# wg-perception/tod

Measured on AMD Instinct MI355X. Metric: frames/sec @ 640x480, 1M-descriptor DB; achieved HBM GB/s on BF-matcher, higher is better.
Workload: dtype fp4 (+-1) x fp4 -> f32 on the matrix cores (exact integers), f32 in the verifier

## Files before the change

tod_amd/csrc/verify.hip:

```cpp
#include <algorithm>
#include <chrono>
#include <atomic>
#include <climits>
#include <cmath>
#include <cstdio>
#include <cstdlib>
#include <cstring>
#include <limits>
#include <map>
#include <memory>
#include <mutex>
#include <thread>
#include <vector>

#include "ctx.h"
#include "depth_rescale.h"
#include "verify_kernels.h"
#include "verify_draw_bits.h"

using namespace tod;

namespace {

#include "verify_launch.h"
#include "verify_prep.h"
#include "verify_draw.h"
#include "verify_clique.h"
#include "verify_eval.h"
#include "verify_growth.h"
#include "verify_sprint.h"


struct VerifyWs {
  DevBuf train, query, qidx, kpxy, phys, samp, bits, sampdeg, nvalid, table, iter_samples, counts, gate_m,
      small, deferred, stacks, kp_bits, clique_adj, adjc_scratch, c_kept, c_offs, c_qpt, c_obj, c_hist, c_goff,
      sprint_status, sprint_stack, c_src, c_cnt;
  HostBuf m_small, m_hist, m_pos, m_counts, m_kp, m_nvalid;
  HostBuf m_sprint, m_sprint_out, m_sprint_kp;
  HostBuf h_small;
};

struct StreamCache;
struct VerifyPool : TodWs {
  static constexpr int kSlot = kWsVerify;
  std::vector<VerifyWs*> slots; std::vector<StreamCache*> streams;
  std::vector<hipEvent_t> side_ev;
  static constexpr size_t kMaxLanes = 17;
  HostBuf args_stage[kMaxLanes]; DevBuf args_dev[kMaxLanes];
  DevBuf kceil; bool kceil_ready = false;
  ~VerifyPool() override;
};
struct SideStreams {
  struct PerDevice {
    std::vector<hipStream_t> st;
    std::atomic<bool> taken[16];
    uint32_t partition = 0;
    PerDevice() { for (auto& t : taken) t.store(false); }
  };
  std::mutex mu;
  std::map<int, PerDevice> by_device;
  hipError_t get(int device, uint32_t n, std::vector<hipStream_t>& out, PerDevice** pd) {
    std::lock_guard<std::mutex> g(mu);
    PerDevice& d = by_device[device];
    const uint32_t part = tod_cu_partition();
    if (d.partition != part) {
      bool in_use = false;
      for (size_t i = 0; i < d.st.size(); ++i) in_use = in_use || d.taken[i].load();
      if (!in_use) {
        for (hipStream_t s0 : d.st) { (void)hipStreamSynchronize(s0); (void)hipStreamDestroy(s0); }
        d.st.clear();
        d.partition = part;
      }
    }
    while (d.st.size() < n) {
      hipStream_t s2;
      const hipError_t e = tod_stream_create(&s2, device, TODHIP_STREAM_LATENCY);
      if (e != hipSuccess) return e;
      d.st.push_back(s2);
    }
    out.assign(d.st.begin(), d.st.begin() + n);
    *pd = &d;
    return hipSuccess;
  }
};
SideStreams g_side_streams;
std::atomic<int> g_batches_in_air{0};

constexpr uint32_t kEvalLdsSmall = 48u * 1024u;
constexpr uint32_t kEvalLdsBig = 160u * 1024u - 512u;
constexpr uint32_t kStackCap = 128u * 1024u;
constexpr uint32_t kMaxEvalWaves = 4096u;

VerifyWs* ws_of(todhip_ctx* ctx, size_t slot = 0) {
  VerifyPool* p = tod_ws<VerifyPool>(ctx);
  while (p->slots.size() <= slot) p->slots.push_back(new VerifyWs());
  return p->slots[slot];
}

struct StreamCache {
  static constexpr uint64_t kSnap = 4096;
  todhip_rng init, gen;
  std::vector<uint32_t> vals;
  std::vector<todhip_rng> snaps;
  explicit StreamCache(const todhip_rng& r) : init(r), gen(r) {}
  bool same_start(const todhip_rng& r) const {
    return r.f == init.f && r.b == init.b && std::memcmp(r.s, init.s, sizeof(init.s)) == 0;
  }
  void extend_to(uint64_t n) {
    while (vals.size() < n) {
      if (vals.size() % kSnap == 0) snaps.push_back(gen);
      vals.push_back(rng_next(gen));
    }
  }
  DevBuf dev;
  uint64_t dev_valid = 0;
  hipError_t ensure_device(uint64_t n, hipStream_t st) {
    extend_to(n);
    if (n <= dev_valid) return hipSuccess;
    const uint64_t want = std::max<uint64_t>(n, 2 * dev_valid);
    extend_to(want);
    if (dev.cap < want * sizeof(uint32_t)) {
      hipError_t e = hipDeviceSynchronize();
      if (e != hipSuccess) return e;
      e = dev.reserve((size_t)want * 2 * sizeof(uint32_t));
      if (e != hipSuccess) return e;
      dev_valid = 0;
    }
    hipError_t e = hipMemcpyAsync(dev.as<uint32_t>() + dev_valid, vals.data() + dev_valid, (size_t)(want - dev_valid) * sizeof(uint32_t),
                                  hipMemcpyHostToDevice, st);
    if (e == hipSuccess) e = hipStreamSynchronize(st);
    if (e == hipSuccess) dev_valid = want;
    return e;
  }
  todhip_rng state_at(uint64_t pos) {
    extend_to(pos + 1);
    todhip_rng g = snaps[pos / kSnap];
    for (uint64_t i = (pos / kSnap) * kSnap; i < pos; ++i) (void)rng_next(g);
    return g;
  }
};

inline double ransac_k(double w) {
  double p_no_outliers = 1.0 - std::pow(w, 3.0);
  p_no_outliers = std::max(std::numeric_limits<double>::epsilon(), p_no_outliers);
  p_no_outliers = std::min(1.0 - std::numeric_limits<double>::epsilon(), p_no_outliers);
  return std::log(1.0 - 0.99) / std::log(p_no_outliers);
}

template <class Launch>
void pick_eval(bool wide, bool deferred, Launch launch) {
  auto extent = [deferred](const EvalArgs& a) { return dim3(deferred ? a.n_deferred : a.it_end - a.it_begin); };
  if (wide) launch(eval_kernel<true, SlotsPtr<EvalArgs>>, eval_kernel<true>, extent);
  else launch(eval_kernel<false, SlotsPtr<EvalArgs>>, eval_kernel<false>, extent);
}

int set_big_lds_once(todhip_ctx* ctx) {
  static std::atomic<bool> done{false};
  if (!done.load(std::memory_order_acquire)) {
    const void* const big[] = {reinterpret_cast<const void*>(eval_kernel<false>), reinterpret_cast<const void*>(eval_kernel<true>),
                               reinterpret_cast<const void*>(eval_kernel<false, SlotsPtr<EvalArgs>>),
                               reinterpret_cast<const void*>(eval_kernel<true, SlotsPtr<EvalArgs>>),
                               reinterpret_cast<const void*>(clique_test_kernel<false>), reinterpret_cast<const void*>(clique_test_kernel<true>),
                               reinterpret_cast<const void*>(chain_kernel)};
    for (const void* f : big) TOD_HIP(hipFuncSetAttribute(f, hipFuncAttributeMaxDynamicSharedMemorySize, (int)kEvalLdsBig));
    TOD_HIP(hipFuncSetAttribute(reinterpret_cast<const void*>(sprint_kernel), hipFuncAttributeMaxDynamicSharedMemorySize,
                                (int)kSprintLds));
    done.store(true, std::memory_order_release);
  }
  return TODHIP_OK;
}

EvalArgs eval_args(const ObjJob& job, VerifyWs* ws, int32_t* counts, uint32_t it_lo, uint32_t it_hi, uint32_t lds_bytes) {
// ... 309 lines not shown
```

tod_amd/csrc/verify_clique.h:

```cpp

struct GateLds {
  u64* adjc;
  u64* mask;
  uint16_t *flist, *cur, *nxt, *tmp;
  uint32_t *C, *deg, *keys;
  uint32_t *S, *SOld, *lbase, *lsize, *lcap;
  uint32_t* trash;
  uint16_t* lstack;
  uint32_t lstack_cap;
};
__host__ __device__ inline uint32_t gate_lds_bytes(uint32_t m) {
  const uint32_t MW = (m + 63u) / 64u, ma = (m + 7u) & ~3u;
  return 8u * m * MW + 8u * MW + 8u * 4u * ma + 4u * 2u * ma + 256u + 64u;
}
__host__ __device__ inline uint32_t gate_small_bytes(uint32_t m) {
  const uint32_t MW = (m + 63u) / 64u, ma = (m + 7u) & ~3u;
  return 8u * MW + 8u * 4u * ma + 4u * 2u * ma + 256u + 64u;
}
template <bool kExt>
__device__ __forceinline__ GateLds gate_carve(unsigned char* base, uint32_t m, uint32_t lds_bytes, u64* ext_adjc = nullptr, uint32_t rows = 0) {
  const uint32_t MW = (m + 63u) / 64u, ma = (m + 7u) & ~3u;
  if (rows == 0u) rows = m;
  unsigned char* const base0 = base;
  GateLds L;
  if constexpr (kExt) { L.adjc = ext_adjc; } else { L.adjc = reinterpret_cast<u64*>(base); base += 8u * rows * MW; }
  L.mask = reinterpret_cast<u64*>(base); base += 8u * MW;
  L.C = reinterpret_cast<uint32_t*>(base); base += 4u * ma;
  L.deg = reinterpret_cast<uint32_t*>(base); base += 4u * ma;
  L.keys = reinterpret_cast<uint32_t*>(base); base += 4u * ma;
  L.S = reinterpret_cast<uint32_t*>(base); base += 4u * ma;
  L.SOld = reinterpret_cast<uint32_t*>(base); base += 4u * ma;
  L.lbase = reinterpret_cast<uint32_t*>(base); base += 4u * ma;
  L.lsize = reinterpret_cast<uint32_t*>(base); base += 4u * ma;
  L.lcap = reinterpret_cast<uint32_t*>(base); base += 4u * ma;
  L.trash = reinterpret_cast<uint32_t*>(base); base += 256u;
  L.flist = reinterpret_cast<uint16_t*>(base); base += 2u * ma;
  L.cur = reinterpret_cast<uint16_t*>(base); base += 2u * ma;
  L.nxt = reinterpret_cast<uint16_t*>(base); base += 2u * ma;
  L.tmp = reinterpret_cast<uint16_t*>(base); base += 2u * ma;
  uint32_t used = ((uint32_t)(base - base0) + 15u) & ~15u;
  L.lstack = reinterpret_cast<uint16_t*>(base0 + used);
  L.lstack_cap = lds_bytes > used ? (lds_bytes - used) / 2u : 0u;
  return L;
}

struct LevelStack { uint16_t* lds; uint32_t lds_cap; uint16_t* glob; };
__device__ __forceinline__ uint16_t stk_get(const LevelStack& s, uint32_t i) {
  return i < s.lds_cap ? s.lds[i] : s.glob[i - s.lds_cap];
}
__device__ __forceinline__ void stk_put(const LevelStack& s, uint32_t i, uint16_t v) {
  if (i < s.lds_cap) s.lds[i] = v; else s.glob[i - s.lds_cap] = v;
}

__device__ __forceinline__ bool row_test(u64 roww, uint32_t h) {
  const u64 wv = shfl64(roww, h >> 6);
  return (wv >> (h & 63u)) & 1ull;
}

constexpr uint32_t kRegChunks = 8;
constexpr uint32_t kSortChunks = 16;

template <uint32_t NCH>
__device__ __forceinline__ void rank_sort_regs(uint16_t* list, const uint32_t* deg, uint32_t r) {
  const uint32_t l = lane_id();
  uint32_t kreg[NCH], rank[NCH];
#pragma unroll
  for (uint32_t c = 0; c < NCH; ++c) {
    const uint32_t i = c * 64u + l;
    kreg[c] = i < r ? ((deg[i] << 16) | list[i]) : 0u;
    rank[c] = 0u;
  }
#pragma unroll
  for (uint32_t cj = 0; cj < NCH; ++cj) {
    const uint32_t cnt = cj * 64u < r ? min(64u, r - cj * 64u) : 0u;
    for (uint32_t lj = 0; lj < cnt; ++lj) {
      const uint32_t kj = rdlane(kreg[cj], lj);
#pragma unroll
      for (uint32_t c = 0; c < NCH; ++c) rank[c] += (kj > kreg[c]) ? 1u : 0u;
    }
  }
  __syncthreads();
#pragma unroll
  for (uint32_t c = 0; c < NCH; ++c)
    if (c * 64u + l < r) list[rank[c]] = (uint16_t)(kreg[c] & 0xFFFFu);
  __syncthreads();
}

template <bool kWide>
__device__ __forceinline__ void rank_sort_desc(uint16_t* list, uint16_t* tmp, const uint32_t* deg, uint32_t r, uint32_t* keys) {
  const uint32_t l = lane_id();
  if (r <= kRegChunks * 64u) {
    switch ((r + 63u) / 64u) {
      case 0: case 1: rank_sort_regs<1>(list, deg, r); break;
      case 2: rank_sort_regs<2>(list, deg, r); break;
      case 3: rank_sort_regs<3>(list, deg, r); break;
      case 4: rank_sort_regs<4>(list, deg, r); break;
      case 5: rank_sort_regs<5>(list, deg, r); break;
      case 6: rank_sort_regs<6>(list, deg, r); break;
      case 7: rank_sort_regs<7>(list, deg, r); break;
      default: rank_sort_regs<8>(list, deg, r); break;
    }
    return;
  }
  if constexpr (kWide) {
    if (r <= kSortChunks * 64u) {
      switch ((r + 63u) / 64u) {
        case 9: rank_sort_regs<9>(list, deg, r); break;
        case 10: rank_sort_regs<10>(list, deg, r); break;
        case 11: rank_sort_regs<11>(list, deg, r); break;
        case 12: rank_sort_regs<12>(list, deg, r); break;
        case 13: case 14: rank_sort_regs<14>(list, deg, r); break;
        default: rank_sort_regs<16>(list, deg, r); break;
      }
      return;
    }
  }
  for (uint32_t i = l; i < r; i += 64u) keys[i] = (deg[i] << 16) | list[i];
  __syncthreads();
  for (uint32_t i0 = 0; i0 < r; i0 += 64u) {
    const uint32_t i = i0 + l;
    const uint32_t mine = i < r ? keys[i] : 0u;
    uint32_t rank = 0;
    for (uint32_t j = 0; j < r; ++j) rank += keys[j] > mine;
    if (i < r) tmp[rank] = (uint16_t)(mine & 0xFFFFu);
  }
  __syncthreads();
  for (uint32_t i = l; i < r; i += 64u) list[i] = tmp[i];
  __syncthreads();
}

__device__ __forceinline__ void degrees_in_list(const GateLds& L, const uint16_t* list, uint32_t r, uint32_t MW) {
  const uint32_t l = lane_id();
  if (l < MW) L.mask[l] = 0ull;
  __syncthreads();
  for (uint32_t i = l; i < r; i += 64u) atomicOr(&L.mask[list[i] >> 6], 1ull << (list[i] & 63u));
  __syncthreads();
  for (uint32_t i = l; i < r; i += 64u) {
    const u64* row = L.adjc + (size_t)list[i] * MW;
    uint32_t d = 0;
    for (uint32_t w = 0; w < MW; ++w) d += (uint32_t)__popcll(row[w] & L.mask[w]);
    L.deg[i] = d;
  }
  __syncthreads();
}

template <uint32_t MWT>
__device__ __forceinline__ bool colour_first_fit64(const GateLds& L, uint16_t* list, uint32_t r) {
  typedef uint32_t u32x16 __attribute__((ext_vector_type(MWT <= 8u ? 16 : 32)));
  const uint32_t l = lane_id();
  u32x16 cls = {};
  uint32_t rec = l << 16;
  uint32_t* const my_trash = L.trash + l;
  for (uint32_t c0 = 0; c0 < r; c0 += 64u) {
    const uint32_t cnt = min(64u, r - c0);
    const uint32_t vmine = (uint32_t)list[min(c0 + l, r - 1u)];
    const uint32_t voff = vmine * (MWT * 8u);
    auto place = [&](const u64 (&row)[MWT], u64 (&next)[MWT], uint32_t li) {
      const uint32_t v = rdlane(vmine, li);
      {
        const u64* g = reinterpret_cast<const u64*>(reinterpret_cast<const unsigned char*>(L.adjc) + rdlane(voff, (li + 1u) & 63u));
#pragma unroll
        for (uint32_t w = 0; w < MWT; ++w) next[w] = g[w];
      }
      uint32_t hit32 = (uint32_t)row[0] & cls[0];
      {
        const uint32_t rh = (uint32_t)(row[0] >> 32), ch = cls[1];
        asm("v_and_or_b32 %0, %1, %2, %0" : "+v"(hit32) : "v"(rh), "v"(ch));
      }
#pragma unroll
      for (uint32_t w = 1; w < MWT; ++w) {
        const uint32_t rl = (uint32_t)row[w], rh = (uint32_t)(row[w] >> 32), cl = cls[2u * w], ch = cls[2u * w + 1u];
        asm("v_and_or_b32 %0, %1, %2, %0" : "+v"(hit32) : "v"(rl), "v"(cl));
        asm("v_and_or_b32 %0, %1, %2, %0" : "+v"(hit32) : "v"(rh), "v"(ch));
      }
      const u64 fm = __ballot(hit32 == 0u);
      const uint32_t below = __builtin_amdgcn_mbcnt_hi((uint32_t)(fm >> 32), __builtin_amdgcn_mbcnt_lo((uint32_t)fm, 0u));
      const uint32_t lw = hit32 == 0u ? below : 1u;
      const bool join = lw == 0u;
      uint32_t* const dst = join ? (L.keys + (c0 + li)) : my_trash;
      *dst = rec;
      rec += join ? 1u : 0u;
      cls[v >> 5] |= join ? (1u << (v & 31u)) : 0u;
    };
    u64 rowA[MWT], rowB[MWT];
    {
      const u64* g = L.adjc + (size_t)rdlane(vmine, 0u) * MWT;
#pragma unroll
      for (uint32_t w = 0; w < MWT; ++w) rowA[w] = g[w];
    }
    uint32_t li = 0;
    for (; li + 2u <= cnt; li += 2u) {
      place(rowA, rowB, li);
      place(rowB, rowA, li + 1u);
    }
    if (li < cnt) place(rowA, rowB, li);
  }
  const uint32_t cnt0 = rec & 0xFFFFu;
  const uint32_t incl0 = wave_incl_scan(cnt0), total0 = uni(__shfl(incl0, 63));
  if (total0 != r) return false;
  const uint32_t base0 = incl0 - cnt0;
  __syncthreads();
  for (uint32_t i = l; i < r + 63u - ((r + 63u) & 63u); i += 64u) {
    const uint32_t rec = i < r ? L.keys[i] : 0u;
    const uint32_t k = rec >> 16;
    const uint32_t b = __shfl(base0, k & 63u);
    if (i < r) {
      const uint32_t pos = b + (rec & 0xFFFFu);
      L.tmp[pos] = list[i];
      L.C[pos] = k + 1u;
    }
  }
  __syncthreads();
  for (uint32_t i = l; i < r; i += 64u) list[i] = L.tmp[i];
  __syncthreads();
  return true;
}

template <uint32_t MWT, bool WIDE>
__device__ __forceinline__ bool colour_first_fit(const GateLds& L, uint16_t* list, uint32_t r) {
  const uint32_t l = lane_id();
  u64 cls0[MWT], cls1[WIDE ? MWT : 1];
#pragma unroll
  for (uint32_t w = 0; w < MWT; ++w) cls0[w] = 0ull;
#pragma unroll
  for (uint32_t w = 0; w < (WIDE ? MWT : 1); ++w) cls1[w] = 0ull;
  uint32_t cnt0 = 0u, cnt1 = 0u;
  bool wide = false, overflow = false;
  for (uint32_t c0 = 0; c0 < r; c0 += 64u) {
    const uint32_t cnt = min(64u, r - c0);
    const uint32_t vmine = (c0 + l) < r ? (uint32_t)list[c0 + l] : 0u;
    uint32_t rec = 0u;
    auto place = [&](const u64 (&row)[MWT], u64 (&next)[MWT], uint32_t li) {
      const uint32_t v = rdlane(vmine, li);
      {
        const u64* g = L.adjc + (size_t)rdlane(vmine, min(li + 1u, cnt - 1u)) * MWT;
#pragma unroll
        for (uint32_t w = 0; w < MWT; ++w) next[w] = g[w];
      }
      u64 hit = 0ull;
#pragma unroll
      for (uint32_t w = 0; w < MWT; ++w) hit |= row[w] & cls0[w];
      const u64 free0 = __ballot(hit == 0ull);
      uint32_t k = 0u;
      bool second = false;
      if (free0 != 0ull) {
        k = (uint32_t)__ffsll((long long)free0) - 1u;
      } else if (WIDE) {
        wide = true; second = true;
        u64 hit1 = 0ull;
#pragma unroll
        for (uint32_t w = 0; w < (WIDE ? MWT : 1); ++w) hit1 |= row[w] & cls1[w];
        const u64 free1 = __ballot(hit1 == 0ull);
        if (free1 == 0ull) overflow = true; else k = (uint32_t)__ffsll((long long)free1) - 1u;
      } else {
        overflow = true;
      }
      const uint32_t vw = v >> 6;
      const u64 bit = 1ull << (v & 63u);
      const uint32_t idx = second ? rdlane(cnt1, k) : rdlane(cnt0, k);
      if (l == k) {
        if (!second) {
          cnt0 += 1u;
#pragma unroll
          for (uint32_t w = 0; w < MWT; ++w)
            if (vw == w) { cls0[w] |= bit; asm volatile("" ::: "memory"); }
        } else if (WIDE) {
          cnt1 += 1u;
#pragma unroll
          for (uint32_t w = 0; w < (WIDE ? MWT : 1); ++w)
            if (vw == w) { cls1[w] |= bit; asm volatile("" ::: "memory"); }
        }
      }
      if (l == li) rec = ((second ? k + 64u : k) << 16) | idx;
    };
    u64 rowA[MWT], rowB[MWT];
    {
      const u64* g = L.adjc + (size_t)rdlane(vmine, 0u) * MWT;
#pragma unroll
      for (uint32_t w = 0; w < MWT; ++w) rowA[w] = g[w];
    }
    uint32_t li = 0;
    for (; li + 2u <= cnt && !overflow; li += 2u) {
      place(rowA, rowB, li);
      place(rowB, rowA, li + 1u);
    }
    if (li < cnt && !overflow) place(rowA, rowB, li);
    if (overflow) return false;
    if (c0 + l < r) L.keys[c0 + l] = rec;
  }
  const uint32_t incl0 = wave_incl_scan(cnt0), total0 = uni(__shfl(incl0, 63));
  const uint32_t base0 = incl0 - cnt0;
  uint32_t base1 = 0u;
  if (wide) { const uint32_t incl1 = wave_incl_scan(cnt1); base1 = total0 + incl1 - cnt1; }
  __syncthreads();
  for (uint32_t i = l; i < r + 63u - ((r + 63u) & 63u); i += 64u) {
    const uint32_t rec = i < r ? L.keys[i] : 0u;
    const uint32_t k = rec >> 16;
    uint32_t b = __shfl(base0, k & 63u);
    if (wide) { const uint32_t b1 = __shfl(base1, k & 63u); b = k >= 64u ? b1 : b; }
    if (i < r) {
      const uint32_t pos = b + (rec & 0xFFFFu);
      L.tmp[pos] = list[i];
      L.C[pos] = k + 1u;
    }
  }
  __syncthreads();
  for (uint32_t i = l; i < r; i += 64u) list[i] = L.tmp[i];
  __syncthreads();
  return true;
}

template <bool kWide>
__device__ __forceinline__ void colour_sort(const GateLds& L, uint16_t* list, uint32_t r, uint32_t MW, uint32_t qmax, uint32_t qsz) {
  const uint32_t l = lane_id();
  const int min_k = max(1, (int)qmax - (int)qsz + 1);
  if (min_k >= 2) {
    if (l == 0) L.C[r - 1] = 0u;
    __syncthreads();
    return;
  }
  if (r <= 2u) {
    if (l == 0) {
      L.C[0] = 1u;
      if (r == 2u) {
        const uint32_t a = list[0], b = list[1];
        L.C[1] = ((L.adjc[(size_t)a * MW + (b >> 6)] >> (b & 63u)) & 1ull) ? 2u : 1u;
      }
    }
    __syncthreads();
    return;
  }
  if (MW <= 8u) {
    bool done = false;
    switch (MW) {
      case 1: done = colour_first_fit64<1>(L, list, r) || colour_first_fit<1, true>(L, list, r); break;
      case 2: done = colour_first_fit64<2>(L, list, r) || colour_first_fit<2, true>(L, list, r); break;
      case 3: done = colour_first_fit64<3>(L, list, r) || colour_first_fit<3, true>(L, list, r); break;
      case 4: done = colour_first_fit64<4>(L, list, r) || colour_first_fit<4, true>(L, list, r); break;
      case 5: done = colour_first_fit64<5>(L, list, r) || colour_first_fit<5, true>(L, list, r); break;
      case 6: done = colour_first_fit64<6>(L, list, r) || colour_first_fit<6, true>(L, list, r); break;
      case 7: done = colour_first_fit64<7>(L, list, r) || colour_first_fit<7, true>(L, list, r); break;
      default: done = colour_first_fit64<8>(L, list, r) || colour_first_fit<8, true>(L, list, r); break;
    }
    if (done) return;
  }
  if constexpr (kWide) {
    if (MW > 8u && MW <= 16u) {
      bool done = false;
      switch (MW) {
        case 9: done = colour_first_fit64<9>(L, list, r) || colour_first_fit<9, true>(L, list, r); break;
        case 10: done = colour_first_fit64<10>(L, list, r) || colour_first_fit<10, true>(L, list, r); break;
        case 11: done = colour_first_fit64<11>(L, list, r) || colour_first_fit<11, true>(L, list, r); break;
        case 12: done = colour_first_fit64<12>(L, list, r) || colour_first_fit<12, true>(L, list, r); break;
        case 13: done = colour_first_fit64<13>(L, list, r) || colour_first_fit<13, true>(L, list, r); break;
        case 14: done = colour_first_fit64<14>(L, list, r) || colour_first_fit<14, true>(L, list, r); break;
        case 15: done = colour_first_fit64<15>(L, list, r) || colour_first_fit<15, true>(L, list, r); break;
        default: done = colour_first_fit64<16>(L, list, r) || colour_first_fit<16, true>(L, list, r); break;
      }
      if (done) return;
    }
  }
  const uint32_t nchunks = (r + 63u) / 64u;
  u64 uncol = 0ull;
  if (l < nchunks) uncol = (l * 64u + 64u <= r) ? ~0ull : ((1ull << (r - l * 64u)) - 1ull);
  uint32_t k = 1, outpos = 0;
  while (__ballot(uncol != 0ull) != 0ull) {
    u64 Q = uncol;
    while (true) {
      const u64 balQ = __ballot(Q != 0ull);
      if (balQ == 0ull) break;
      const uint32_t ll = (uint32_t)__ffsll((long long)balQ) - 1u;
      const u64 wq = shfl64(Q, ll);
      const uint32_t bit = uni((uint32_t)__ffsll((long long)wq) - 1u);
      const uint32_t g = uni(list[ll * 64u + bit]);
      if (l == 0) { L.tmp[outpos] = (uint16_t)g; L.C[outpos] = k; }
      ++outpos;
      if (l == ll) { uncol &= ~(1ull << bit); Q &= ~(1ull << bit); }
      const u64* grow = L.adjc + (size_t)g * MW;
      for (uint32_t c = 0; c < nchunks; ++c) {
        if (!((balQ >> c) & 1ull)) continue;
        const uint32_t pos = c * 64u + l;
        bool adj = false;
        if (pos < r) { const uint32_t h = list[pos]; adj = (grow[h >> 6] >> (h & 63u)) & 1ull; }
        const u64 bal = __ballot(adj);
        if (l == c) Q &= ~bal;
      }
    }
    ++k;
  }
  __syncthreads();
  for (uint32_t i = l; i < r; i += 64u) list[i] = L.tmp[i];
  __syncthreads();
}

template <bool kWide, bool kGate>
__device__ __forceinline__ uint32_t clique_search(GateLds L, uint32_t m, uint32_t minimal_size, uint16_t* gstack, uint32_t stack_cap,
                                  int* err, uint32_t* steps_out, uint32_t* prof = nullptr, const uint16_t* vertices = nullptr) {
  const uint32_t l = lane_id();
  const LevelStack stack = {L.lstack, L.lstack_cap, gstack};
  stack_cap += L.lstack_cap;
  const uint32_t MW = (m + 63u) / 64u;
  uint32_t dmax = 0;
  for (uint32_t i = l; i < m; i += 64u) { L.cur[i] = vertices ? vertices[i] : (uint16_t)i; dmax = max(dmax, L.deg[i]); }
#pragma unroll
  for (int o = 32; o > 0; o >>= 1) dmax = max(dmax, (uint32_t)__shfl_xor((int)dmax, o));
  const uint32_t max_degree = uni(dmax);
  __syncthreads();
  rank_sort_desc<kWide>(L.cur, L.tmp, L.deg, m, L.keys);
  __syncthreads();
  for (uint32_t i = l; i < m; i += 64u) L.C[i] = i < max_degree ? i + 1u : max_degree + 1u;
  for (uint32_t i = l; i < m + 2u; i += 64u) { L.S[i] = 0u; L.SOld[i] = 0u; }
  for (uint32_t i = l; i < m; i += 64u) stk_put(stack, i, L.cur[i]);
  if (l == 0) { L.lbase[1] = 0u; L.lsize[1] = m; L.lcap[1] = m; }
  __syncthreads();

  uint32_t level = 1, qsz = 0, qmax = 0, top = m;
  int all_steps = 1;
  uint32_t pf_isect = 0, pf_sort = 0, pf_col = 0, pf_vfull = 0, pf_big = 0, pf_vbig = 0;
  auto in_lds = [&](uint32_t b, uint32_t n) { return b + n <= stack.lds_cap; };
  uint16_t* cur = in_lds(0u, m) ? stack.lds : L.cur;
  const uint32_t ma = (m + 7u) & ~3u;
  auto frame_word = [&](uint32_t lvl) -> uint32_t { return l < 5u ? (L.S + (size_t)l * ma)[lvl] : 0u; };
  uint32_t sz = m, S_cur = 0u, base_cur = 0u, cap_cur = m;
  while (true) {
    bool ret = false;
    if (sz == 0u) {
      ret = true;
    } else {
      const uint32_t pv = cur[sz - 1u];
      const uint32_t cv = top > 0u ? L.C[top - 1u] : 0u;
      const uint32_t p = uni(pv), c = uni(cv);
      if (qsz + c > qmax) {
        ++qsz;
        const u64* prow = L.adjc + (size_t)p * MW;
        const long long pt0 = prof ? clock64() : 0;
        const uint32_t nb = base_cur + cap_cur;
        const bool in_place = in_lds(nb, sz);
        uint16_t* const nxt = in_place ? stack.lds + nb : (cur == L.cur ? L.nxt : L.cur);
        uint32_t rp = 0;
        for (uint32_t i0 = 0; i0 < sz; i0 += 64u) {
          const uint32_t i = i0 + l;
          uint32_t h = 0;
          bool adj = false;
          if (i < sz) { h = cur[i]; adj = (prow[h >> 6] >> (h & 63u)) & 1ull; }
          const u64 bal = __ballot(adj);
          if (adj) nxt[rp + (uint32_t)__popcll(bal & ((1ull << l) - 1ull))] = (uint16_t)h;
          rp += (uint32_t)__popcll(bal);
        }
        rp = uni(rp);
        __syncthreads();
        const long long pt1 = prof ? clock64() : 0;
        pf_isect += (uint32_t)(pt1 - pt0);
        if constexpr (kGate) {
          if (rp > 0u && qmax < minimal_size && qsz >= minimal_size && (uint32_t)all_steps + rp + 1u <= (uint32_t)kStepCap) { qmax = qsz + 1u; break; }
        }
        if (rp > 0u) {
          if ((uint64_t)S_cur * 40ull < (uint64_t)all_steps) {
            degrees_in_list(L, nxt, rp, MW);
            rank_sort_desc<kWide>(nxt, L.tmp, L.deg, rp, L.keys);
          }
          const long long pt2 = prof ? clock64() : 0;
          pf_sort += (uint32_t)(pt2 - pt1);
          colour_sort<kWide>(L, nxt, rp, MW, qmax, qsz);
          if (prof) {
            const uint32_t dt = (uint32_t)(clock64() - pt2);
            pf_col += dt;
            if ((int)qmax - (int)qsz + 1 < 2) { pf_vfull += rp; if (rp > 64u) { pf_big += dt; pf_vbig += rp; } }
          }
          S_cur += 1u;
          ++all_steps;
          if (all_steps > kStepCap) {
            ret = true;
          } else {
            if (nb + rp > stack_cap) { *err = 1; break; }
            if (!in_place)
              for (uint32_t i = l; i < rp; i += 64u) stk_put(stack, nb + i, nxt[i]);
            const uint32_t child = frame_word(level + 1u);
            if (l == 0) { L.S[level] = S_cur; L.lsize[level] = sz; L.lbase[level] = base_cur; L.lcap[level] = cap_cur; }
            const uint32_t s_child = rdlane(child, 0u), sold_child = rdlane(child, 1u);
            ++level;
            cur = nxt;
            if (qmax >= minimal_size) {
              if (l == 0) L.S[level] = s_child;
              S_cur = s_child; sz = rp; base_cur = nb; cap_cur = rp;
              ret = true;
            } else {
              if (l == 0) L.SOld[level] = S_cur;
              S_cur = s_child + S_cur - sold_child;
              sz = rp; base_cur = nb; cap_cur = rp;
              __syncthreads();
              continue;
            }
          }
        } else {
          if (qsz > qmax) {
            qmax = qsz;
            if (qmax >= minimal_size) {
              if constexpr (kGate) break;
              ret = true;
            }
          }
          if (!ret) --qsz;
        }
      } else {
        ret = true;
      }
      if (!ret) {
        --sz;
        if (top > 0u) --top;
        continue;
      }
    }
    if (level == 1u) break;
    if (l == 0) L.S[level] = S_cur;
    --level;
    --qsz;
    if (top > 0u) --top;
    __syncthreads();
    const uint32_t fw = frame_word(level);
    S_cur = rdlane(fw, 0u); base_cur = rdlane(fw, 2u); sz = rdlane(fw, 3u) - 1u; cap_cur = rdlane(fw, 4u);
    if (in_lds(base_cur, cap_cur)) {
      cur = stack.lds + base_cur;
    } else {
      cur = L.cur;
      for (uint32_t i = l; i < sz; i += 64u) cur[i] = stk_get(stack, base_cur + i);
    }
    __syncthreads();
  }
  if (steps_out) *steps_out = (uint32_t)all_steps;
  if (prof && l == 0) { prof[0] = pf_isect; prof[1] = pf_sort; prof[2] = pf_col; prof[3] = pf_big; prof[4] = pf_vbig; prof[5] = pf_vfull; }
  return qmax;
}

template <bool kGate>
__global__ __launch_bounds__(128) void clique_test_kernel(const u64* adj, uint32_t m, uint32_t minimal_size,
                                                         uint16_t* stack, uint32_t stack_cap, uint32_t lds_bytes,
                                                         uint32_t* out) {
  extern __shared__ __align__(16) unsigned char lds_raw[];
  const uint32_t l = lane_id();
  GateLds L = gate_carve<false>(lds_raw, m, lds_bytes);
  const uint32_t MW = (m + 63u) / 64u;
  for (uint32_t i = l; i < m * MW; i += 64u) L.adjc[i] = adj[i];
  __syncthreads();
  for (uint32_t g = l; g < m; g += 64u) {
    uint32_t d = 0;
    for (uint32_t w = 0; w < MW; ++w) d += (uint32_t)__popcll(L.adjc[(size_t)g * MW + w]);
    L.deg[g] = d;
  }
  __syncthreads();
  int err = 0;
  uint32_t steps = 0;
  const uint32_t q = clique_search<true, kGate>(L, m, minimal_size, stack, stack_cap, &err, &steps);
  if (l == 0) { out[0] = q; out[1] = (uint32_t)err; out[2] = steps; }
}
```

tod_amd/csrc/verify_eval.h:

```cpp

constexpr uint32_t kAdjcScratchWords = 256u * 1024u;

struct EvalArgs {
  ObjJob job;
  const uint32_t* iter_samples;
  uint32_t it_begin, it_end;
  int32_t* counts;
  uint32_t* gate_m;
  uint32_t* work;
  EvalStatus* status;
  uint32_t* deferred;
  uint16_t* stacks;
  uint32_t stack_cap;
  uint32_t lds_bytes;
  uint32_t from_deferred;
  uint32_t n_deferred;
  u64* adjc_scratch;
  uint32_t* dbg;
  uint32_t dbg_stride;
  uint32_t stop_level;
  const uint32_t* n_items_dev;
};

template <bool kExt, bool kWide, int kSlices>
// ... 90 lines not shown
          L.deg[grow] = d;
        }
      }
    } else if (W <= 64u) {
      constexpr uint32_t kRows = 8;
      for (uint32_t g0 = 0; g0 < m; g0 += kRows) {
        u64 rw[kRows];
#pragma unroll
        for (uint32_t j = 0; j < kRows; ++j) {
          const uint32_t g = g0 + j;
          rw[j] = (g < m && l < W) ? job.samp[(size_t)uni(L.flist[g < m ? g : 0u]) * W + l] : 0ull;
        }
#pragma unroll
        for (uint32_t j = 0; j < kRows; ++j) {
          const uint32_t g = g0 + j;
          if (g < m) {
            uint32_t d = 0;
            for (uint32_t c = 0; c < MW; ++c) {
              const uint32_t pos = c * 64u + l;
              const uint32_t h = pos < m ? L.flist[pos] : 0u;
              const bool adj = row_test(rw[j], h) && pos < m;
              const u64 bal = __ballot(adj);
              if (l == 0) L.adjc[(size_t)g * MW + c] = bal;
              d += (uint32_t)__popcll(bal);
            }
            if (l == 0) L.deg[g] = d;
          }
        }
      }
    } else {
      for (uint32_t g = 0; g < m; ++g) {
        const u64* row = job.samp + (size_t)uni(L.flist[g]) * W;
        uint32_t d = 0;
        for (uint32_t c = 0; c < MW; ++c) {
          const uint32_t pos = c * 64u + l;
          bool adj = false;
          if (pos < m) { const uint32_t h = L.flist[pos]; adj = (row[h >> 6] >> (h & 63u)) & 1ull; }
          const u64 bal = __ballot(adj);
          if (l == 0) L.adjc[(size_t)g * MW + c] = bal;
          d += (uint32_t)__popcll(bal);
        }
        if (l == 0) L.deg[g] = d;
      }
    }
  }
  __syncthreads();
  const long long t_adjc = A.dbg ? clock64() : 0;
  if (A.dbg) {
    uint32_t* d = A.dbg + (size_t)it * A.dbg_stride;
    if (l == 0) { d[0] = cnt; d[1] = m; }
    for (uint32_t g = l; g < m && 2u + 2u * g + 1u < A.dbg_stride; g += 64u) { d[2 + 2 * g] = L.flist[g]; d[3 + 2 * g] = L.deg[g]; }
  }
  bool any = false;
  for (uint32_t g = l; g < m; g += 64u) any = any || L.deg[g] > kGateMinimal;
  if (bad_index) {
    result = INT_MIN;
  } else if (A.stop_level != 0u) {
    result = -(int32_t)m;
  } else if (__ballot(any) == 0ull) {
    result = 0;
  } else {
    int err = 0;
    uint32_t steps = 0;
    uint32_t* prof = (A.dbg && A.dbg_stride >= 16u) ? A.dbg + (size_t)it * A.dbg_stride + (A.dbg_stride - 12u) : nullptr;
    const uint32_t q = clique_search<kWide, true>(L, m, kGateMinimal, stack, A.stack_cap, &err, &steps, prof, ident ? L.flist : nullptr);
    if (A.dbg && l == 0 && A.dbg_stride >= 8u) {
      uint32_t* d = A.dbg + (size_t)it * A.dbg_stride + (A.dbg_stride - 6u);
      d[0] = (uint32_t)(t_flist - t_start); d[1] = (uint32_t)(t_adjc - t_flist);
      d[2] = (uint32_t)(clock64() - t_adjc); d[3] = steps; d[4] = q;
    }
    if (err) {
      if (l == 0) atomicExch(&A.status->error, 1u);
      result = INT_MIN;
    } else if (q <= kGateMinimal) {
      result = 0;
    }
    if (l == 0) atomicAdd(&A.status->gate_calls, 1u);
  }
  __syncthreads();
  return result;
}

template <bool kWide, class H = Slots<EvalArgs>>
__global__ __launch_bounds__(128) void eval_kernel(H SL) {
  TOD_LATENCY_PRIO();
  const EvalArgs& A = SL.a[blockIdx.y];
  extern __shared__ __align__(16) unsigned char lds_raw[];
  const uint32_t l = lane_id();
  const ObjJob& job = A.job;
  const uint32_t W = job.W;
  uint16_t* stack = A.stacks + (size_t)blockIdx.x * A.stack_cap;
  uint32_t n_items = A.from_deferred ? A.n_deferred : (A.it_end - A.it_begin);
  if (A.n_items_dev) n_items = min(n_items, uni(*A.n_items_dev));
  {
    const uint32_t item = blockIdx.x;
    if (item >= n_items) return;
    const uint32_t it = uni(A.from_deferred ? A.deferred[item] : (A.it_begin + item));
    const uint32_t s0 = uni(A.iter_samples[3 * it]), s1 = uni(A.iter_samples[3 * it + 1]),
                   s2 = uni(A.iter_samples[3 * it + 2]);
    if (s0 >= job.n || s1 >= job.n || s2 >= job.n) {
      if (l == 0) { atomicExch(&A.status->error, 3u); A.counts[it] = INT_MIN; }
      return;
    }
    typedef WaveBitsT<kWide ? kWPL : 1> Bits;
    Bits P;
    wb_load(P, job.phys + (size_t)s0 * W, W);
    wb_and(P, job.phys + (size_t)s1 * W, W);
    wb_and(P, job.phys + (size_t)s2 * W, W);
    wb_and(P, job.valid, W);
    wb_and(P, job.finite, W);
    const uint32_t cnt = wb_count(P) + 3u;
    int32_t result = (int32_t)cnt;
    uint32_t m_diag = 0;
    if (cnt > kGateMinimal && A.stop_level != 2u) {
      Bits F = P;
      wb_set(F, s0); wb_set(F, s1); wb_set(F, s2);
      wb_and(F, job.deg7, W);
      const uint32_t m = wb_count(F);
      m_diag = m;
      if (m <= kGateMinimal) {
        result = 0;
      } else if (gate_lds_bytes(m) > A.lds_bytes &&
                 !(A.from_deferred && A.adjc_scratch && gate_small_bytes(m) <= A.lds_bytes &&
                   m * ((m + 63u) / 64u) <= kAdjcScratchWords)) {
        if (A.from_deferred) {
          if (l == 0) atomicExch(&A.status->error, 2u);
          result = INT_MIN;
        } else {
          if (l == 0) A.deferred[atomicAdd(&A.status->n_deferred, 1u)] = it;
          result = INT_MIN + 1;
        }
      } else {
        result = gate_lds_bytes(m) > A.lds_bytes ? gate_eval<true, kWide>(A, F, m, it, cnt, lds_raw, stack)
                                                 : gate_eval<false, kWide>(A, F, m, it, cnt, lds_raw, stack);
      }
    }
    if (l == 0) {
      if (result != INT_MIN + 1) A.counts[it] = result;
      if (A.gate_m) A.gate_m[it] = m_diag;
    }
  }
}
```

tod_amd/csrc/verify_kernels.h:

```cpp
#pragma once

#include <hip/hip_runtime.h>

#include <cstddef>
#include <cstdint>

namespace tod {

typedef unsigned long long u64;

constexpr int kMaxWords = 512;
constexpr int kWPL = 8;
constexpr uint32_t kMaxSampleChecks = 1000;
constexpr uint32_t kGateMinimal = 7;
constexpr int kStepCap = 100000;

struct ObjJob {
  uint32_t n, W;
  const float* train;
  const float* query;
  const uint32_t* qidx;
  const float* kpxy;
  u64* phys;
  u64* samp;
  u64* finite;
  u64* valid;
  u64* deg7;
  uint32_t* sampdeg;
};

struct DrawEntry { uint32_t status, consumed, s0, s1, s2, pad; };
enum { DRAW_FAIL = 0, DRAW_OK = 1, DRAW_OVERFLOW = 2 };

struct ChainOut {
  uint32_t n_done;
  uint32_t pos_end;
  uint32_t attempts;
  uint32_t flag;
};

struct EvalStatus {
  uint32_t error;
  uint32_t gate_calls;
  uint32_t n_deferred;
  uint32_t pad_;
  uint32_t detail_g, detail_value, detail_m, detail_it;
};

struct GrowthOut {
  float R[9], T[3];
  uint32_t n_match_inliers;
  uint32_t n_kp_inliers;
  uint32_t passes;
  uint32_t n_model_inliers;
};

struct ClusterCtl {
  uint32_t error, pad1_[3];
  uint32_t n_kept, pad5_[3];
};

template <class Tail>
struct SlotWords {
  uint32_t pad0_;
  ChainOut chain;
  uint32_t prep[3];
  uint32_t eval_work;
  uint32_t pad9_[3];
  EvalStatus eval;
  uint32_t pad20_[12];
  GrowthOut growth;
  uint32_t pad48_[12];
  Tail tail;
};
struct SlotCtlTail { uint32_t pad60_[4]; };
struct SlotMailTail { ClusterCtl cluster; uint32_t pad68_[60]; };
typedef SlotWords<SlotCtlTail> SlotCtl;
typedef SlotWords<SlotMailTail> SlotMail;
constexpr uint32_t kMailSmallWords = 128u;

#define TOD_WORD_AT(T, member, word) static_assert(offsetof(T, member) == (word) * 4u, #T "::" #member " moved")
TOD_WORD_AT(EvalStatus, error, 0); TOD_WORD_AT(EvalStatus, gate_calls, 1); TOD_WORD_AT(EvalStatus, n_deferred, 2);
TOD_WORD_AT(EvalStatus, detail_g, 4); TOD_WORD_AT(EvalStatus, detail_value, 5); TOD_WORD_AT(EvalStatus, detail_m, 6);
TOD_WORD_AT(EvalStatus, detail_it, 7);
TOD_WORD_AT(ClusterCtl, error, 0); TOD_WORD_AT(ClusterCtl, n_kept, 4);
TOD_WORD_AT(SlotCtl, chain, 1); TOD_WORD_AT(SlotCtl, prep, 5); TOD_WORD_AT(SlotCtl, eval_work, 8); TOD_WORD_AT(SlotCtl, eval, 12);
TOD_WORD_AT(SlotCtl, growth, 32); TOD_WORD_AT(SlotCtl, tail, 60);
TOD_WORD_AT(SlotMail, chain, 1); TOD_WORD_AT(SlotMail, prep, 5); TOD_WORD_AT(SlotMail, eval_work, 8); TOD_WORD_AT(SlotMail, eval, 12);
TOD_WORD_AT(SlotMail, growth, 32); TOD_WORD_AT(SlotMail, tail.cluster.error, 60); TOD_WORD_AT(SlotMail, tail.cluster.n_kept, 64);
static_assert(sizeof(EvalStatus) == 8 * 4 && sizeof(ChainOut) == 4 * 4 && sizeof(GrowthOut) == 16 * 4 && sizeof(ClusterCtl) == 8 * 4, "mailbox layout");
static_assert(sizeof(SlotCtl) == 64 * 4 && sizeof(SlotMail) == kMailSmallWords * 4, "mailbox layout");

#undef TOD_WORD_AT

__device__ __forceinline__ uint32_t lane_id() { return threadIdx.x & 63u; }

__device__ __forceinline__ uint32_t uni(uint32_t v) { return (uint32_t)__builtin_amdgcn_readfirstlane((int)v); }

__device__ __forceinline__ uint32_t rdlane(uint32_t v, uint32_t lane) {
  return (uint32_t)__builtin_amdgcn_readlane((int)v, (int)lane);
}
__device__ __forceinline__ u64 rdlane64(u64 v, uint32_t lane) {
  return ((u64)rdlane((uint32_t)(v >> 32), lane) << 32) | rdlane((uint32_t)v, lane);
}

__device__ __forceinline__ uint32_t wave_sum(uint32_t v) {
#pragma unroll
  for (int off = 32; off > 0; off >>= 1) v += __shfl_xor(v, off);
  return uni(v);
}
__device__ __forceinline__ uint32_t wave_incl_scan(uint32_t v) {
  const uint32_t l = lane_id();
#pragma unroll
  for (int d = 1; d < 64; d <<= 1) {
    uint32_t t = __shfl_up(v, d);
    if (l >= (uint32_t)d) v += t;
  }
  return v;
}
__device__ __forceinline__ u64 shfl64(u64 v, uint32_t src) {
  uint32_t lo = __shfl((uint32_t)v, src), hi = __shfl((uint32_t)(v >> 32), src);
  return ((u64)hi << 32) | lo;
}
__device__ __forceinline__ uint32_t nth_set_bit(u64 w, uint32_t n) {
  for (uint32_t i = 0; i < n; ++i) w &= w - 1;
  return (uint32_t)__ffsll((long long)w) - 1u;
}

template <int kSlices = kWPL>
struct WaveBitsT {
  u64 w[kSlices];
};
typedef WaveBitsT<> WaveBits;
template <int kSlices>
__device__ __forceinline__ void wb_load(WaveBitsT<kSlices>& b, const u64* p, uint32_t W) {
  const uint32_t l = lane_id();
#pragma unroll
  for (int j = 0; j < kSlices; ++j) b.w[j] = (j * 64u + l) < W ? p[j * 64u + l] : 0ull;
}
template <int kSlices>
__device__ __forceinline__ void wb_and(WaveBitsT<kSlices>& b, const u64* p, uint32_t W) {
  const uint32_t l = lane_id();
#pragma unroll
  for (int j = 0; j < kSlices; ++j) b.w[j] &= (j * 64u + l) < W ? p[j * 64u + l] : 0ull;
}
template <int kSlices>
__device__ __forceinline__ uint32_t wb_count(const WaveBitsT<kSlices>& b) {
  uint32_t c = 0;
#pragma unroll
  for (int j = 0; j < kSlices; ++j) c += (uint32_t)__popcll(b.w[j]);
  return wave_sum(c);
}
template <int kSlices>
__device__ __forceinline__ void wb_clear(WaveBitsT<kSlices>& b, uint32_t v) {
  const uint32_t word = v >> 6, l = lane_id();
#pragma unroll
  for (int j = 0; j < kSlices; ++j)
    if (word == j * 64u + l) b.w[j] &= ~(1ull << (v & 63u));
}
template <int kSlices>
__device__ __forceinline__ void wb_set(WaveBitsT<kSlices>& b, uint32_t v) {
  const uint32_t word = v >> 6, l = lane_id();
#pragma unroll
  for (int j = 0; j < kSlices; ++j)
    if (word == j * 64u + l) b.w[j] |= (1ull << (v & 63u));
}
template <int kSlices>
__device__ __forceinline__ uint32_t wb_select(const WaveBitsT<kSlices>& b, uint32_t idx) {
  idx = uni(idx);
  uint32_t result = 0xFFFFFFFFu;
#pragma unroll
  for (int j = 0; j < kSlices; ++j) {
    const uint32_t c = (uint32_t)__popcll(b.w[j]);
    const uint32_t incl = wave_incl_scan(c);
    const uint32_t total = uni(__shfl(incl, 63));
    if (result == 0xFFFFFFFFu) {
      if (idx < total) {
        const bool mine = (incl - c) <= idx && idx < incl;
        const u64 bal = __ballot(mine);
        const uint32_t owner = (uint32_t)__ffsll((long long)bal) - 1u;
        const uint32_t bit = mine ? nth_set_bit(b.w[j], idx - (incl - c)) : 0u;
        result = (j * 64u + owner) * 64u + uni(__shfl(bit, owner));
      } else {
        idx -= total;
      }
    }
  }
  return result;
}

__device__ __forceinline__ float dist_sq3(const float* a, const float* b) {
  float t0 = a[0] - b[0], t1 = a[1] - b[1], t2 = a[2] - b[2];
  return t0 * t0 + t1 * t1 + t2 * t2;
}
__device__ __forceinline__ double norm3d(float x, float y, float z) {
  return sqrt((double)x * (double)x + (double)y * (double)y + (double)z * (double)z);
}

}
// ... 1 lines not shown
```

tod_amd/csrc/verify_launch.h:

```cpp

constexpr uint32_t kMaxSlots = 16;
constexpr uint32_t kManySlots = 36;
template <class A, uint32_t N = kMaxSlots> struct Slots { A a[N]; };
template <class A> struct SlotsPtr { const A* a; };

struct CopyArgs { const uint32_t* src; uint32_t* dst; uint32_t n; };

constexpr uint32_t kWideSlots = 32;
constexpr uint32_t kCopySlots = 160;
__global__ __launch_bounds__(256) void copy_words_kernel(Slots<CopyArgs, kCopySlots> S) {
  const CopyArgs& a = S.a[blockIdx.y];
  for (uint32_t i = blockIdx.x * 256u + threadIdx.x; i < a.n; i += gridDim.x * 256u) a.dst[i] = a.src ? a.src[i] : 0u;
}

inline int tod_debug_level() { static const int lv = [] { const char* e = getenv("TODHIP_DEBUG"); return e ? std::max(1, atoi(e)) : 0; }(); return lv; }
inline bool tod_debug() { return tod_debug_level() > 0; }
inline double dbg_us() {
  static const std::chrono::steady_clock::time_point t0 = std::chrono::steady_clock::now();
  return std::chrono::duration<double, std::micro>(std::chrono::steady_clock::now() - t0).count();
}
inline int dbg_thread() { static std::atomic<int> next{0}; thread_local int id = next.fetch_add(1); return id; }
#define TOD_DBG2(...) do { if (tod_debug_level() > 1) { fprintf(stderr, "[todhip %.0f] ", dbg_us()); fprintf(stderr, __VA_ARGS__); fputc('\n', stderr); fflush(stderr); } } while (0)
#define TOD_DBG(...) do { if (tod_debug()) { char b_[512]; int n_ = snprintf(b_, sizeof(b_), "[todhip %.0f] ", dbg_us()); n_ += snprintf(b_ + n_, sizeof(b_) - n_, __VA_ARGS__); \
    snprintf(b_ + std::min<int>(n_, (int)sizeof(b_) - 16), 16, " {t%d}\n", dbg_thread()); fputs(b_, stderr); } } while (0)

template <uint32_t N = kMaxSlots, class A, class Kern, class Extent>
void launch_list(hipStream_t st, Kern kern, const std::vector<A>& v, uint32_t block, uint32_t lds, int slot_dim, Extent extent) {
  static_assert(sizeof(Slots<A, N>) <= 4096, "kernel arguments are limited to 4 KB");
  for (size_t i0 = 0; i0 < v.size(); i0 += N) {
    const uint32_t n = (uint32_t)std::min<size_t>(N, v.size() - i0);
    Slots<A, N> S;
    std::memset(&S, 0, sizeof(S));
    uint32_t gx = 1, gy = 1;
    for (uint32_t i = 0; i < n; ++i) {
      S.a[i] = v[i0 + i];
      const dim3 e = extent(v[i0 + i]);
      gx = std::max(gx, e.x); gy = std::max(gy, e.y);
    }
    dim3 grid;
    if (slot_dim == 0) grid = dim3(n);
    else if (slot_dim == 1) grid = dim3(gx, n);
    else grid = dim3(gx, gy, n);
    hipLaunchKernelGGL(kern, grid, dim3(block), lds, st, S);
  }
}
```

Before: 25120.

## Tune verifier clique kernels: occupancy hints, bpermute scans, pruned eval path

```diff
diff --git a/tod_amd/csrc/verify.hip b/tod_amd/csrc/verify.hip
--- a/tod_amd/csrc/verify.hip
+++ b/tod_amd/csrc/verify.hip
@@ -88,6 +88,7 @@
 
 constexpr uint32_t kEvalLdsSmall = 48u * 1024u;
 constexpr uint32_t kEvalLdsBig = 160u * 1024u - 512u;
+static_assert(gate_lds_bytes(8u * 64u) <= kEvalLdsBig, "eval_kernel<false> has no third tier: its largest graph must fit the deferred pass's LDS");
 constexpr uint32_t kStackCap = 128u * 1024u;
 constexpr uint32_t kMaxEvalWaves = 4096u;
 
diff --git a/tod_amd/csrc/verify_clique.h b/tod_amd/csrc/verify_clique.h
--- a/tod_amd/csrc/verify_clique.h
+++ b/tod_amd/csrc/verify_clique.h
@@ -9,7 +9,7 @@
   uint16_t* lstack;
   uint32_t lstack_cap;
 };
-__host__ __device__ inline uint32_t gate_lds_bytes(uint32_t m) {
+__host__ __device__ constexpr uint32_t gate_lds_bytes(uint32_t m) {
   const uint32_t MW = (m + 63u) / 64u, ma = (m + 7u) & ~3u;
   return 8u * m * MW + 8u * MW + 8u * 4u * ma + 4u * 2u * ma + 256u + 64u;
 }
@@ -62,7 +62,7 @@
 
 template <uint32_t NCH>
 __device__ __forceinline__ void rank_sort_regs(uint16_t* list, const uint32_t* deg, uint32_t r) {
-  const uint32_t l = lane_id();
+  const uint32_t l = lane_here();
   uint32_t kreg[NCH], rank[NCH];
 #pragma unroll
   for (uint32_t c = 0; c < NCH; ++c) {
@@ -88,7 +88,7 @@
 
 template <bool kWide>
 __device__ __forceinline__ void rank_sort_desc(uint16_t* list, uint16_t* tmp, const uint32_t* deg, uint32_t r, uint32_t* keys) {
-  const uint32_t l = lane_id();
+  const uint32_t l = lane_here();
   if (r <= kRegChunks * 64u) {
     switch ((r + 63u) / 64u) {
       case 0: case 1: rank_sort_regs<1>(list, deg, r); break;
@@ -130,7 +130,7 @@
 }
 
 __device__ __forceinline__ void degrees_in_list(const GateLds& L, const uint16_t* list, uint32_t r, uint32_t MW) {
-  const uint32_t l = lane_id();
+  const uint32_t l = lane_here();
   if (l < MW) L.mask[l] = 0ull;
   __syncthreads();
   for (uint32_t i = l; i < r; i += 64u) atomicOr(&L.mask[list[i] >> 6], 1ull << (list[i] & 63u));
@@ -147,7 +147,7 @@
 template <uint32_t MWT>
 __device__ __forceinline__ bool colour_first_fit64(const GateLds& L, uint16_t* list, uint32_t r) {
   typedef uint32_t u32x16 __attribute__((ext_vector_type(MWT <= 8u ? 16 : 32)));
-  const uint32_t l = lane_id();
+  const uint32_t l = lane_here();
   u32x16 cls = {};
   uint32_t rec = l << 16;
   uint32_t* const my_trash = L.trash + l;
@@ -196,7 +196,7 @@
     if (li < cnt) place(rowA, rowB, li);
   }
   const uint32_t cnt0 = rec & 0xFFFFu;
-  const uint32_t incl0 = wave_incl_scan(cnt0), total0 = uni(__shfl(incl0, 63));
+  const uint32_t incl0 = wave_incl_scan(cnt0, l), total0 = rdlane(incl0, 63u);
   if (total0 != r) return false;
   const uint32_t base0 = incl0 - cnt0;
   __syncthreads();
@@ -218,7 +218,7 @@
 
 template <uint32_t MWT, bool WIDE>
 __device__ __forceinline__ bool colour_first_fit(const GateLds& L, uint16_t* list, uint32_t r) {
-  const uint32_t l = lane_id();
+  const uint32_t l = lane_here();
   u64 cls0[MWT], cls1[WIDE ? MWT : 1];
 #pragma unroll
   for (uint32_t w = 0; w < MWT; ++w) cls0[w] = 0ull;
@@ -230,27 +230,31 @@
     const uint32_t cnt = min(64u, r - c0);
     const uint32_t vmine = (c0 + l) < r ? (uint32_t)list[c0 + l] : 0u;
     uint32_t rec = 0u;
-    auto place = [&](const u64 (&row)[MWT], u64 (&next)[MWT], uint32_t li) {
+    auto place = [&](u64 (&row)[MWT], uint32_t li) {
       const uint32_t v = rdlane(vmine, li);
+      uint32_t hit = 0u, hit1 = 0u;
+      auto fold = [](uint32_t& acc, u64 r, u64 c) {
+        const uint32_t rl = (uint32_t)r, rh = (uint32_t)(r >> 32), cl = (uint32_t)c, ch = (uint32_t)(c >> 32);
+        asm("v_and_or_b32 %0, %1, %2, %0" : "+v"(acc) : "v"(rl), "v"(cl));
+        asm("v_and_or_b32 %0, %1, %2, %0" : "+v"(acc) : "v"(rh), "v"(ch));
+      };
+#pragma unroll
+      for (uint32_t w = 0; w < MWT; ++w) fold(hit, row[w], cls0[w]);
+#pragma unroll
+      for (uint32_t w = 0; w < (WIDE ? MWT : 1); ++w) fold(hit1, row[w], cls1[w]);
+      const u64 free0 = __ballot(hit == 0u), free1 = __ballot(hit1 == 0u);
+      asm volatile("" : : "s"(free0), "s"(free1) : "memory");
       {
         const u64* g = L.adjc + (size_t)rdlane(vmine, min(li + 1u, cnt - 1u)) * MWT;
 #pragma unroll
-        for (uint32_t w = 0; w < MWT; ++w) next[w] = g[w];
-      }
-      u64 hit = 0ull;
-#pragma unroll
-      for (uint32_t w = 0; w < MWT; ++w) hit |= row[w] & cls0[w];
-      const u64 free0 = __ballot(hit == 0ull);
+        for (uint32_t w = 0; w < MWT; ++w) row[w] = g[w];
+      }
       uint32_t k = 0u;
       bool second = false;
       if (free0 != 0ull) {
         k = (uint32_t)__ffsll((long long)free0) - 1u;
       } else if (WIDE) {
         wide = true; second = true;
-        u64 hit1 = 0ull;
-#pragma unroll
-        for (uint32_t w = 0; w < (WIDE ? MWT : 1); ++w) hit1 |= row[w] & cls1[w];
-        const u64 free1 = __ballot(hit1 == 0ull);
         if (free1 == 0ull) overflow = true; else k = (uint32_t)__ffsll((long long)free1) - 1u;
       } else {
         overflow = true;
@@ -273,25 +277,20 @@
       }
       if (l == li) rec = ((second ? k + 64u : k) << 16) | idx;
     };
-    u64 rowA[MWT], rowB[MWT];
+    u64 row[MWT];
     {
       const u64* g = L.adjc + (size_t)rdlane(vmine, 0u) * MWT;
 #pragma unroll
-      for (uint32_t w = 0; w < MWT; ++w) rowA[w] = g[w];
-    }
-    uint32_t li = 0;
-    for (; li + 2u <= cnt && !overflow; li += 2u) {
-      place(rowA, rowB, li);
-      place(rowB, rowA, li + 1u);
-    }
-    if (li < cnt && !overflow) place(rowA, rowB, li);
+      for (uint32_t w = 0; w < MWT; ++w) row[w] = g[w];
+    }
+    for (uint32_t li = 0; li < cnt && !overflow; ++li) place(row, li);
     if (overflow) return false;
     if (c0 + l < r) L.keys[c0 + l] = rec;
   }
-  const uint32_t incl0 = wave_incl_scan(cnt0), total0 = uni(__shfl(incl0, 63));
+  const uint32_t incl0 = wave_incl_scan(cnt0, l), total0 = rdlane(incl0, 63u);
   const uint32_t base0 = incl0 - cnt0;
   uint32_t base1 = 0u;
-  if (wide) { const uint32_t incl1 = wave_incl_scan(cnt1); base1 = total0 + incl1 - cnt1; }
+  if (wide) { const uint32_t incl1 = wave_incl_scan(cnt1, l); base1 = total0 + incl1 - cnt1; }
   __syncthreads();
   for (uint32_t i = l; i < r + 63u - ((r + 63u) & 63u); i += 64u) {
     const uint32_t rec = i < r ? L.keys[i] : 0u;
@@ -312,7 +311,7 @@
 
 template <bool kWide>
 __device__ __forceinline__ void colour_sort(const GateLds& L, uint16_t* list, uint32_t r, uint32_t MW, uint32_t qmax, uint32_t qsz) {
-  const uint32_t l = lane_id();
+  const uint32_t l = lane_here();
   const int min_k = max(1, (int)qmax - (int)qsz + 1);
   if (min_k >= 2) {
     if (l == 0) L.C[r - 1] = 0u;
@@ -396,14 +395,14 @@
 template <bool kWide, bool kGate>
 __device__ __forceinline__ uint32_t clique_search(GateLds L, uint32_t m, uint32_t minimal_size, uint16_t* gstack, uint32_t stack_cap,
                                   int* err, uint32_t* steps_out, uint32_t* prof = nullptr, const uint16_t* vertices = nullptr) {
-  const uint32_t l = lane_id();
+  const uint32_t l = lane_here();
   const LevelStack stack = {L.lstack, L.lstack_cap, gstack};
   stack_cap += L.lstack_cap;
   const uint32_t MW = (m + 63u) / 64u;
   uint32_t dmax = 0;
   for (uint32_t i = l; i < m; i += 64u) { L.cur[i] = vertices ? vertices[i] : (uint16_t)i; dmax = max(dmax, L.deg[i]); }
 #pragma unroll
-  for (int o = 32; o > 0; o >>= 1) dmax = max(dmax, (uint32_t)__shfl_xor((int)dmax, o));
+  for (uint32_t o = 32; o > 0; o >>= 1) dmax = max(dmax, (uint32_t)__builtin_amdgcn_ds_bpermute((int)((l ^ o) << 2), (int)dmax));
   const uint32_t max_degree = uni(dmax);
   __syncthreads();
   rank_sort_desc<kWide>(L.cur, L.tmp, L.deg, m, L.keys);
@@ -537,7 +536,7 @@
                                                          uint16_t* stack, uint32_t stack_cap, uint32_t lds_bytes,
                                                          uint32_t* out) {
   extern __shared__ __align__(16) unsigned char lds_raw[];
-  const uint32_t l = lane_id();
+  const uint32_t l = lane_here();
   GateLds L = gate_carve<false>(lds_raw, m, lds_bytes);
   const uint32_t MW = (m + 63u) / 64u;
   for (uint32_t i = l; i < m * MW; i += 64u) L.adjc[i] = adj[i];
diff --git a/tod_amd/csrc/verify_eval.h b/tod_amd/csrc/verify_eval.h
--- a/tod_amd/csrc/verify_eval.h
+++ b/tod_amd/csrc/verify_eval.h
@@ -196,9 +196,9 @@
 }
 
 template <bool kWide, class H = Slots<EvalArgs>>
-__global__ __launch_bounds__(128) void eval_kernel(H SL) {
+__global__ __launch_bounds__(128) __attribute__((amdgpu_waves_per_eu(kWide ? 1 : 5))) void eval_kernel(H SL) {
   TOD_LATENCY_PRIO();
-  const EvalArgs& A = SL.a[blockIdx.y];
+  const EvalArgs& A = slot_args(SL, blockIdx.y);
   extern __shared__ __align__(16) unsigned char lds_raw[];
   const uint32_t l = lane_id();
   const ObjJob& job = A.job;
@@ -235,7 +235,7 @@
       if (m <= kGateMinimal) {
         result = 0;
       } else if (gate_lds_bytes(m) > A.lds_bytes &&
-                 !(A.from_deferred && A.adjc_scratch && gate_small_bytes(m) <= A.lds_bytes &&
+                 !(kWide && A.from_deferred && A.adjc_scratch && gate_small_bytes(m) <= A.lds_bytes &&
                    m * ((m + 63u) / 64u) <= kAdjcScratchWords)) {
         if (A.from_deferred) {
           if (l == 0) atomicExch(&A.status->error, 2u);
@@ -245,8 +245,11 @@
           result = INT_MIN + 1;
         }
       } else {
-        result = gate_lds_bytes(m) > A.lds_bytes ? gate_eval<true, kWide>(A, F, m, it, cnt, lds_raw, stack)
-                                                 : gate_eval<false, kWide>(A, F, m, it, cnt, lds_raw, stack);
+        if constexpr (kWide)
+          result = gate_lds_bytes(m) > A.lds_bytes ? gate_eval<true, kWide>(A, F, m, it, cnt, lds_raw, stack)
+                                                   : gate_eval<false, kWide>(A, F, m, it, cnt, lds_raw, stack);
+        else
+          result = gate_eval<false, kWide>(A, F, m, it, cnt, lds_raw, stack);
       }
     }
     if (l == 0) {
diff --git a/tod_amd/csrc/verify_kernels.h b/tod_amd/csrc/verify_kernels.h
--- a/tod_amd/csrc/verify_kernels.h
+++ b/tod_amd/csrc/verify_kernels.h
@@ -94,6 +94,11 @@
 #undef TOD_WORD_AT
 
 __device__ __forceinline__ uint32_t lane_id() { return threadIdx.x & 63u; }
+__device__ __forceinline__ uint32_t lane_here() {
+  uint32_t l = lane_id();
+  asm volatile("" : "+v"(l));
+  return l;
+}
 
 __device__ __forceinline__ uint32_t uni(uint32_t v) { return (uint32_t)__builtin_amdgcn_readfirstlane((int)v); }
 
@@ -115,6 +120,14 @@
   for (int d = 1; d < 64; d <<= 1) {
     uint32_t t = __shfl_up(v, d);
     if (l >= (uint32_t)d) v += t;
+  }
+  return v;
+}
+__device__ __forceinline__ uint32_t wave_incl_scan(uint32_t v, uint32_t l) {
+#pragma unroll
+  for (uint32_t d = 1; d < 64u; d <<= 1) {
+    const uint32_t t = (uint32_t)__builtin_amdgcn_ds_bpermute((int)((l - d) << 2), (int)v);
+    if (l >= d) v += t;
   }
   return v;
 }
diff --git a/tod_amd/csrc/verify_launch.h b/tod_amd/csrc/verify_launch.h
--- a/tod_amd/csrc/verify_launch.h
+++ b/tod_amd/csrc/verify_launch.h
@@ -3,6 +3,18 @@
 constexpr uint32_t kManySlots = 36;
 template <class A, uint32_t N = kMaxSlots> struct Slots { A a[N]; };
 template <class A> struct SlotsPtr { const A* a; };
+template <class A, uint32_t N>
+__device__ __forceinline__ const A& slot_args(const Slots<A, N>& S, uint32_t i) { return S.a[i]; }
+template <class A>
+__device__ __forceinline__ A slot_args(const SlotsPtr<A>& S, uint32_t i) {
+  static_assert(sizeof(A) % 4u == 0 && alignof(A) >= 4u, "copied as dwords");
+  typedef const __attribute__((address_space(4))) uint32_t* ConstWords;
+  ConstWords src = (ConstWords)(S.a + i);
+  union { A a; uint32_t w[sizeof(A) / 4u]; } u;
+#pragma unroll
+  for (uint32_t k = 0; k < sizeof(A) / 4u; ++k) u.w[k] = src[k];
+  return u.a;
+}
 
 struct CopyArgs { const uint32_t* src; uint32_t* dst; uint32_t n; };
 
```

Result: no change. 25300, median of 5 (+0.7%).
